# vadimkantorov/convasr

Hardware: AMD Instinct MI355X
Metric: audio-seconds/sec/node (fwd+bwd+CTC) at bs64x15s (higher is better)
Workload: dtype bf16

## Files before the change

### convasr_amd/_lib.py

```python
import ctypes
import os

import torch

_HERE = os.path.dirname(os.path.abspath(__file__))
LIB_PATH = os.environ.get('CONVASR_HIP_LIB') or os.path.join(_HERE, 'libconvasr_hip.so')

F32, BF16, I16, F16 = 0, 1, 2, 3
LOSS_SCALER_FLOATS = 8
ACT_NONE, ACT_RELU, ACT_HARDTANH, ACT_LEAKY_RELU = 0, 1, 2, 3
PACK_FWD, PACK_DGRAD = 0, 1
W_REFERENCE, W_KMAJOR = 0, 1
METRIC_CHARS, METRIC_WORDS = 0, 1
METRIC_MAX_LEN = 16383

c_int, c_i64, c_u64, c_f32, c_p = ctypes.c_int, ctypes.c_int64, ctypes.c_uint64, ctypes.c_float, ctypes.c_void_p

_SIGNATURES = dict(
	convasr_abi_version = (c_int, []),
	convasr_last_error = (ctypes.c_char_p, []),
	convasr_convert_layout = (c_int, [c_p, c_int, c_i64, c_i64, c_i64, c_p, c_int, c_i64, c_i64, c_i64, c_int, c_int, c_int, c_p]),
	convasr_signal_absmax = (c_int, [c_p, c_int, c_int, c_int, c_p, c_p]),
	convasr_logmel_fwd = (c_int, [c_p, c_int, c_p, c_p, c_p, c_int, c_p, c_p, c_p, c_int, c_int, c_int, c_int, c_int, c_f32, c_p]),
	convasr_instnorm_fwd = (c_int, [c_p, c_int, c_i64, c_i64, c_i64, c_p, c_int, c_i64, c_i64, c_i64, c_p, c_int, c_int, c_int, c_int, c_f32, c_p]),
	convasr_instnorm_running_fwd = (c_int, [c_p, c_int, c_i64, c_i64, c_i64, c_p, c_int, c_i64, c_i64, c_i64, c_int, c_int, c_int, c_int, c_f32, c_p, c_p, c_p, c_f32, c_int, c_p, c_p]),
	convasr_output_lengths = (c_int, [c_p, c_int, c_int, c_p, c_p]),
	convasr_conv_cout_pad = (c_int, [c_int]),
	convasr_pack_conv_weight = (c_int, [c_p, c_p, c_p, c_int, c_int, c_int, c_int, c_int, c_p]),
	convasr_fold2_geometry = (c_int, [c_int, c_int, ctypes.POINTER(c_int), ctypes.POINTER(c_int)]),
	convasr_fold2_pack_weight = (c_int, [c_p, c_int, c_p, c_int, c_int, c_int, c_int, c_int, c_p]),
	convasr_fold2_unfold_wgrad = (c_int, [c_p, c_p, c_int, c_int, c_int, c_int, c_int, c_int, c_p]),
	convasr_conv1d_fwd = (c_int, [c_p, c_p, c_p, c_int, c_int, c_int, c_int, c_int, c_int, c_int, c_int, c_int, c_int, c_int, c_p, c_p, c_p, c_p, c_int, c_f32, c_f32, c_p, c_p, c_p]),
	convasr_conv_stats_max_rows = (c_int, [c_int, c_int]),
	convasr_grouped_conv1d_fwd = (c_int, [c_p, c_p, c_i64, c_i64, c_i64, c_p, c_p, c_int, c_int, c_int, c_int, c_int, c_int, c_int, c_int, c_int, c_int, c_int, c_p]),
	convasr_grouped_conv1d_dgrad = (c_int, [c_p, c_p, c_p, c_i64, c_i64, c_i64, c_p, c_int, c_int, c_int, c_int, c_int, c_int, c_int, c_int, c_int, c_int, c_p]),
	convasr_grouped_conv1d_wgrad_workspace_bytes = (c_i64, [c_int, c_int, c_int, c_int, c_int]),
	convasr_grouped_conv1d_wgrad = (c_int, [c_p, c_p, c_p, c_p, c_i64, c_i64, c_i64, c_p, c_p, c_int, c_int, c_int, c_int, c_int, c_int, c_int, c_int, c_int, c_int, c_int, c_p]),
	convasr_reduce_rows = (c_int, [c_p, c_int, c_int, c_p, c_p]),
	convasr_debug_set_conv_v2 = (c_int, [c_int]),
	convasr_conv1d_wgrad_workspace_bytes = (c_i64, [c_int, c_int, c_int, c_int, c_int, c_int, c_int, c_int]),
	convasr_conv1d_wgrad = (c_int, [c_p, c_p, c_p, c_p, c_p, c_int, c_int, c_int, c_int, c_int, c_int, c_int, c_int, c_int, c_int, c_int, c_int, c_p]),
	convasr_bn_finalize = (c_int, [c_p, c_int, c_i64, c_p, c_p, c_p, c_p, c_f32, c_f32, c_p, c_p, c_p, c_p, c_int, c_p, c_p]),
	convasr_bn_eval_scale_shift = (c_int, [c_p, c_p, c_p, c_p, c_f32, c_p, c_p, c_int, c_p]),
	convasr_bn_act_fwd = (c_int, [c_p, c_p, c_int, c_p, c_p, c_int, c_p, c_p, c_p, c_int, c_f32, c_f32, c_f32, c_u64, c_u64, c_p, c_p, c_int, c_int, c_int, c_p, c_p]),
	convasr_bn_bwd_workspace_bytes = (c_i64, [c_int, c_int, c_int]),
	convasr_bn_act_bwd_reduce = (c_int, [c_p, c_p, c_p, c_int, c_p, c_p, c_p, c_p, c_int, c_p, c_p, c_p, c_p, c_p, c_p, c_int, c_f32, c_f32, c_f32, c_u64, c_u64, c_p, c_p, c_p, c_p, c_p, c_p, c_p, c_p, c_int, c_int, c_int, c_int, c_p, c_p]),
	convasr_bn_act_bwd_apply = (c_int, [c_p, c_p, c_p, c_int, c_p, c_int, c_p, c_p, c_int, c_f32, c_f32, c_f32, c_u64, c_u64, c_p, c_p, c_int, c_int, c_int, c_p, c_p]),
	convasr_bn_bwd_apply = (c_int, [c_p, c_p, c_p, c_int, c_p, c_p, c_p, c_p, c_p, c_p, c_int, c_int, c_int, c_int, c_p]),
	convasr_log_softmax_fwd = (c_int, [c_p, c_p, c_i64, c_int, c_p]),
	convasr_log_softmax_bwd = (c_int, [c_p, c_p, c_p, c_i64, c_int, c_p]),
	convasr_ctc_workspace_bytes = (c_i64, [c_int, c_int, c_int]),
	convasr_ctc_loss = (c_int, [c_p, c_p, c_p, c_p, c_p, c_p, c_p, c_int, c_int, c_int, c_int, c_int, c_p]),
	convasr_scale_rows = (c_int, [c_p, c_p, c_p, c_i64, c_p, c_int, c_i64, c_p]),
	convasr_loss_head = (c_int, [c_p, c_p, c_i64, c_p, c_int, c_f32, c_p, c_p, c_p, c_p, c_f32, c_p]),
	convasr_entropy = (c_int, [c_p, c_p, c_p, c_int, c_int, c_int, c_f32, c_p]),
	convasr_weighted_mean_entropy = (c_int, [c_p, c_p, c_p, c_int, c_int, c_int, c_int, c_f32, c_p]),
	convasr_argmax = (c_int, [c_p, c_p, c_i64, c_int, c_p]),
	convasr_sumsq_workspace_bytes = (c_i64, []),
	convasr_sumsq = (c_int, [c_p, c_i64, c_p, c_p, c_p, c_f32, c_p, c_p]),
	convasr_sgd_step = (c_int, [c_p, c_p, c_p, c_p, c_i64, c_p, c_f32, c_f32, c_f32, c_f32, c_int, c_int, c_p, c_f32, c_p, c_int, c_p, c_p, c_p, c_p]),
	convasr_adamw_step = (c_int, [c_p, c_p, c_p, c_p, c_i64, c_p, c_f32, c_f32, c_f32, c_f32, c_f32, c_f32, c_p, c_p, c_p, c_f32, c_p, c_int, c_p, c_p, c_p, c_p]),
	convasr_conv1d_dgrad_bn_reduce = (c_int, [c_p, c_p, c_p, c_int, c_int, c_int, c_int, c_int, c_int, c_int, c_int, c_int, c_p, c_p, c_p, c_p, c_p, c_int, c_f32, c_f32, c_f32, c_u64, c_u64, c_p, c_p, c_p, c_p, c_p, c_p]),
	convasr_bn_bwd_finalize = (c_int, [c_p, c_int, c_p, c_p, c_p, c_p, c_p, c_p, c_int, c_i64, c_int, c_p]),
	convasr_novograd_step = (c_int, [c_p, c_p, c_p, c_p, c_p, c_p, c_p, c_int, c_i64, c_p, c_int, c_p, c_p, c_f32, c_f32, c_f32, c_f32, c_f32, c_f32, c_int, c_int, c_p, c_p, c_f32, c_p, c_int, c_p, c_p, c_p, c_p]),
	convasr_step_begin = (c_int, [c_p, c_p]),
	convasr_conv1x1_grouped = (c_int, [c_int, c_p, c_p, c_p, c_p, c_p, c_p, c_p, c_p, c_int, c_int, c_int, ctypes.POINTER(c_int), c_p]),
	convasr_add16 = (c_int, [c_p, c_p, c_p, c_i64, c_int, c_p]),
	convasr_bn_bwd_reduce_many_workspace_bytes = (c_i64, [c_int, c_int, c_int, c_int]),
	convasr_bn_bwd_reduce_many = (c_int, [c_p, c_p, c_f32, c_p, c_int, c_p, c_p, c_p, c_p, c_p, c_p, c_p, c_p, c_p, c_int, c_int, c_int, c_int, c_p]),
	convasr_pack_dgrad_item_bytes = (c_int, []),
	convasr_pack_dgrad_grouped = (c_int, [c_p, c_int, c_int, c_p]),
	convasr_bn_finalize_grouped = (c_int, [c_int, c_p, c_int, c_i64, c_p, c_p, c_p, c_p, c_p, c_p, c_p, c_p, c_int, c_p]),
	convasr_bn_bwd_finalize_grouped = (c_int, [c_int, c_p, c_p, c_p, c_p, c_p, c_p, c_p, c_p, c_p, c_i64, c_int, c_p]),
	convasr_bn_bwd_apply_grouped = (c_int, [c_p, c_int, c_p, c_p, c_p, c_int, c_int, c_int, c_int, c_p]),
	convasr_wgrad1x1_grouped_workspace_bytes = (c_i64, [c_int, c_p, c_p, c_int, c_int]),
	convasr_wgrad1x1_grouped = (c_int, [c_int, c_p, c_p, c_p, c_p, c_p, c_p, c_p, c_p, c_int, c_int, c_int, c_p]),
	convasr_copy = (c_int, [c_p, c_p, c_i64, c_p]),
	convasr_colsum_workspace_bytes = (c_i64, [c_i64, c_int]),
	convasr_colsum = (c_int, [c_p, c_int, c_i64, c_int, c_p, c_p, c_int, c_p]),
	convasr_cast_scale = (c_int, [c_p, c_int, c_p, c_int, c_i64, c_f32, c_p]),
	convasr_bn_act_fwd_split3 = (c_int, [c_p, c_p, c_int, c_p, c_p, c_int, c_p, c_p, c_p, c_int, c_f32, c_f32, c_f32, c_u64, c_u64, c_p, c_p, c_int, c_int, c_int, c_p, c_p]),
	convasr_bn_act_bwd_apply_split3 = (c_int, [c_p, c_p, c_p, c_int, c_p, c_int, c_p, c_p, c_int, c_f32, c_f32, c_f32, c_u64, c_u64, c_p, c_p, c_int, c_int, c_int, c_p, c_p]),
	convasr_split3 = (c_int, [c_p, c_p, c_int, c_i64, c_int, c_int, c_p]),
	convasr_pack_conv_weight_split3 = (c_int, [c_p, c_int, c_p, c_p, c_int, c_int, c_int, c_int, c_int, c_p]),
	convasr_bn_act_bwd_apply_to_half = (c_int, [c_p, c_p, c_p, c_int, c_p, c_int, c_p, c_p, c_int, c_f32, c_f32, c_f32, c_u64, c_u64, c_p, c_p, c_int, c_int, c_int, c_p, c_p]),
	convasr_conv1d_fwd_splitk_plan = (c_int, [c_int, c_int, c_int, c_int, c_int, c_int, c_p]),
# ... 239 lines not shown
```

### convasr_amd/csrc/ctc.hip

```cpp
#include "common.h"

#define CTC_NEG (-1e30f)
#define CTC_DEAD (-1e29f)
#define CTC_LOG2E 1.4426950408889634f
#define CTC_LN2 0.6931471805599453
#define CTC_RENORM 8
#define CTC_RENORM_LOG2 3
#define CTC_EMPTY 0xFFFFFFFFu
#ifndef CTC_SPIN_LIMIT
#define CTC_SPIN_LIMIT (1 << 22)
#endif

__device__ __forceinline__ float lse3(float a, float b, float c) {
	const float m = fmaxf(a, fmaxf(b, c));
	const float md = __builtin_amdgcn_fmed3f(a, b, c), lo = fminf(a, fminf(b, c));
	return m + __builtin_amdgcn_logf(1.f + __builtin_amdgcn_exp2f(md - m) + __builtin_amdgcn_exp2f(lo - m));
}
__device__ __forceinline__ float lse2(float a, float b) {
	const float m = __builtin_amdgcn_fmed3f(a, b, INFINITY);
	return m + __builtin_amdgcn_logf(1.f + __builtin_amdgcn_exp2f(__builtin_amdgcn_fmed3f(a, b, -INFINITY) - m));
}

__device__ __forceinline__ float wave_shr1(float v, float fill) {
	return __builtin_bit_cast(float, __builtin_amdgcn_update_dpp(__builtin_bit_cast(int, fill), __builtin_bit_cast(int, v), 0x138, 0xf, 0xf, false));
// ... 194 lines not shown
			const int t = i / (C + 1), c = i - t * (C + 1);
			lpl[i] = c < C ? ctc_floor(lpg[(int64_t)t * C + c] * CTC_LOG2E) : CTC_NEG;
		}
	}
	__syncthreads();
	const int wave = __builtin_amdgcn_readfirstlane(threadIdx.x >> 6);
	const bool fwd = wave < 2;
	CtcSweep q;
	q.lpb = LP_LDS ? lpl : lpg;
	q.tg = targets + (int64_t)b * S_max;
	q.lat = (fwd ? alpha : beta) + (int64_t)b * T * CAP;
	q.off = offs + (((int64_t)(fwd ? 0 : 1) * B + b) * 2 + (wave & 1)) * NB;
	q.edge = edge + (fwd ? 0 : T);
	q.ecum = edge + 3 * T + (fwd ? 0 : NB);
	q.fin = fin; q.fcum = fcum + (wave & 1); q.gave_up = fcum + 2;
	q.T = T; q.C = C; q.Tb = Tb; q.L = L; q.blank = blank; q.cap = CAP; q.lane = threadIdx.x & 63;
	q.s_base = wave == 1 ? 128 * NPH : (wave == 3 ? 128 * NPL : 0);
	if (wave == 0) ctc_sweep<NPH, true, false, LP_LDS>(q);
	else if (wave == 1) ctc_sweep<NPL, true, true, LP_LDS>(q);
	else if (wave == 2) ctc_sweep<NPL, false, true, LP_LDS>(q);
	else ctc_sweep<NPH, false, false, LP_LDS>(q);
	__syncthreads();
	if (threadIdx.x == 0) {
		const float c1 = fcum[L - 1 >= 128 * NPH];
		const float l1 = fin[L - 1], l2 = L >= 2 ? fin[L - 2] + (fcum[L - 2 >= 128 * NPH] - c1) : CTC_NEG;
		const float m = fmaxf(l1, l2);
		const float rem = m + log2f(exp2f(l1 - m) + exp2f(l2 - m));
		nll[b] = fcum[2] != 0.f ? NAN : (m > CTC_DEAD ? (float)(-CTC_LN2 * ((double)c1 + (double)rem)) : INFINITY);
		tot[2 * b] = c1;
		tot[2 * b + 1] = rem;
	}
}

__global__ __launch_bounds__(256) void ctc_grad_kernel(const float* __restrict__ lp, const int64_t* __restrict__ targets, const int64_t* __restrict__ olen,
                                                       const int64_t* __restrict__ ylen, const float* __restrict__ nll, const float* __restrict__ alpha,
                                                       const float* __restrict__ beta, const float* __restrict__ offs, const float* __restrict__ tot, float* __restrict__ grad,
                                                       int B, int T, int C, int S_max, int blank, int t_per_block, int cap, int split_a, int split_b) {
	extern __shared__ float bins[];
	const int NB = T / CTC_RENORM + 1;
	const int b = blockIdx.y, lane = threadIdx.x & 63, wave = threadIdx.x >> 6;
	const int Tb = (int)olen[b], S = (int)ylen[b], L = 2 * S + 1;
	const bool feasible = nll[b] < INFINITY;
	const int64_t* tg = targets + (int64_t)b * S_max;
	float* mybins = bins + wave * C;
	const int t_begin = blockIdx.x * t_per_block, t_end = min(T, t_begin + t_per_block);
	for (int t = t_begin + wave; t < t_end; t += 4) {
		const float* row = lp + ((int64_t)b * T + t) * C;
		float* grow = grad + ((int64_t)b * T + t) * C;
		if (t >= Tb || !feasible) {
			for (int c = lane; c < C; c += 64) grow[c] = 0.f;
			continue;
		}
		for (int c = lane; c < C; c += 64) mybins[c] = 0.f;
		__builtin_amdgcn_s_waitcnt(0xc07f);
		__builtin_amdgcn_wave_barrier();
		const float* ar = alpha + ((int64_t)b * T + t) * cap;
		const float* br = beta + ((int64_t)b * T + t) * cap;
		const float* oa = offs + (int64_t)b * 2 * NB + (t >> CTC_RENORM_LOG2);
		const float* ob = offs + ((int64_t)B + b) * 2 * NB + ((Tb - 1 - t) >> CTC_RENORM_LOG2);
		const float ti = tot[2 * b], tr = tot[2 * b + 1];
		const float oa0 = oa[0] - ti, oa1 = oa[NB] - ti, ob0 = ob[0], ob1 = ob[NB];
		const float lpb = row[blank] * CTC_LOG2E;
		float blank_sum = 0.f;
		for (int s = lane; s < L; s += 64) {
			const float shift = ((s >= split_a ? oa1 : oa0) + (s >= split_b ? ob1 : ob0)) - tr;
			const float ab = ar[s] + br[s];
			if (s & 1) {
				const int c = (int)tg[s >> 1];
				atomicAdd(mybins + c, __builtin_amdgcn_exp2f(ab + (shift - row[c] * CTC_LOG2E)));
			} else blank_sum += __builtin_amdgcn_exp2f(ab + (shift - lpb));
		}
		blank_sum = wave_sum(blank_sum);
		if (lane == 0) atomicAdd(mybins + blank, blank_sum);
		__builtin_amdgcn_s_waitcnt(0xc07f);
		__builtin_amdgcn_wave_barrier();
		for (int c = lane; c < C; c += 64) grow[c] = __expf(row[c]) - mybins[c];
		__builtin_amdgcn_wave_barrier();
	}
}

static int ctc_split(int S_max, int* nph, int* npl) {
	const int pairs = (2 * S_max + 1 + 127) / 128;
	if (pairs > 16) return -1;
	const int p = pairs < 2 ? 2 : pairs;
	*nph = (p + 1) / 2;
	*npl = p / 2;
	return 0;
}

extern "C" int64_t convasr_ctc_workspace_bytes(int B, int T, int S_max) {
	int nph, npl;
	if (ctc_split(S_max, &nph, &npl) < 0) return -1;
	const int NB = T / CTC_RENORM + 1;
	return (2 * (int64_t)B * T * 128 * (nph + npl) + 4 * (int64_t)B * NB + 2 * (int64_t)B) * (int64_t)sizeof(float);
}

extern "C" int convasr_ctc_loss(const float* log_probs, const int64_t* targets, const int64_t* olen, const int64_t* ylen, float* nll, float* grad,
                                void* workspace, int B, int T, int C, int S_max, int blank, void* stream) {
	CONVASR_CHECK_ARG(log_probs && targets && olen && ylen && nll && workspace && B > 0 && T > 0 && C > 1 && S_max >= 0 && blank >= 0 && blank < C, "ctc_loss: bad arguments");
	int nph, npl;
	if (ctc_split(S_max, &nph, &npl) < 0) return convasr_fail(CONVASR_EUNSUPPORTED, "ctc_loss: target length %d > 1023", S_max);
	CONVASR_CHECK_ARG(C <= 8192, "ctc_loss: C %d > 8192", C);
	hipStream_t s = (hipStream_t)stream;
	const int NB = T / CTC_RENORM + 1, cap = 128 * (nph + npl);
	float* alpha = (float*)workspace;
	float* beta = alpha + (int64_t)B * T * cap;
	float* offs = beta + (int64_t)B * T * cap;
	float* tot = offs + 4 * (int64_t)B * NB;
	const int t_per_block = 32;
	dim3 ggrid((T + t_per_block - 1) / t_per_block, B);
	const size_t gsmem = 4 * (size_t)C * sizeof(float);
	const size_t lds_fixed = (size_t)(cap + 4 + ((3 * T + 2 * NB + 3) & ~3)) * sizeof(float), lds_lp = (size_t)T * (C + 1) * sizeof(float);
	CONVASR_CHECK_ARG(lds_fixed <= 159 * 1024, "ctc_loss: T %d too long for the edge slots", T);
	const bool in_lds = lds_fixed + lds_lp <= 159 * 1024;
#define CTC_LAUNCH(NPH, NPL, LDS) do { \
		auto kern = ctc_alpha_beta_kernel<NPH, NPL, LDS>; \
		static unsigned long long set = 0; \
		convasr_allow_160k_lds(reinterpret_cast<const void*>(kern), set); \
		hipLaunchKernelGGL(kern, dim3(B), dim3(256), lds_fixed + (LDS ? lds_lp : 0), s, log_probs, targets, olen, ylen, nll, alpha, beta, offs, tot, B, T, C, S_max, blank); \
	} while (0)
#define CTC_CASE(NPH, NPL) case NPH + NPL: if (in_lds) CTC_LAUNCH(NPH, NPL, true); else CTC_LAUNCH(NPH, NPL, false); break;
	switch (nph + npl) {
		CTC_CASE(1, 1) CTC_CASE(2, 1) CTC_CASE(2, 2) CTC_CASE(3, 2) CTC_CASE(3, 3) CTC_CASE(4, 3) CTC_CASE(4, 4)
		CTC_CASE(5, 4) CTC_CASE(5, 5) CTC_CASE(6, 5) CTC_CASE(6, 6) CTC_CASE(7, 6) CTC_CASE(7, 7) CTC_CASE(8, 7) CTC_CASE(8, 8)
	}
#undef CTC_CASE
#undef CTC_LAUNCH
	if (grad) hipLaunchKernelGGL(ctc_grad_kernel, ggrid, dim3(256), gsmem, s, log_probs, targets, olen, ylen, nll, alpha, beta, offs, tot, grad, B, T, C, S_max, blank, t_per_block, cap, 128 * nph, 128 * npl);
	CONVASR_CHECK_LAUNCH("ctc_loss");
	return 0;
}
```

### convasr_amd/functional.py

```python
import os

import torch

from . import ops, _lib

_pack_cache = {}
_param_epoch = [0]


def bump_param_epoch():
	_param_epoch[0] += 1


def param_version(w):
	return (w._version, w.data_ptr(), _param_epoch[0])


def packed_weight(w, dtype, mode):
	ver = param_version(w)
	ent = _pack_cache.get((id(w), dtype))
	if ent is not None:
		if mode == _lib.PACK_DGRAD:
			if ent['dgr_ver'] == ver:
				return ent['dgr']
# ... 1128 lines not shown
	def forward(ctx, logits):
		lp = ops.log_softmax(ops.as_cl(logits, torch.float32))
		ctx.save_for_backward(lp)
		return lp

	@staticmethod
	def backward(ctx, g):
		lp, = ctx.saved_tensors
		return ops.log_softmax_bwd(g, lp)


class CtcLossFunction(torch.autograd.Function):

	@staticmethod
	def forward(ctx, log_probs, targets, olen, ylen, blank, norm = None):
		lp = ops.as_cl(log_probs, torch.float32)
		need = log_probs.requires_grad
		nll, grad = ops.ctc_loss(lp, targets, olen, ylen, blank, need_grad = need)
		ctx.norm = norm
		if need:
			ctx.save_for_backward(grad)
		if norm is None:
			return nll
		if norm.dtype == torch.int64 and norm.ndim == 1 and norm.device == nll.device:
			return ops.scale_rows(nll, None, norm)
		return nll / norm

	@staticmethod
	def backward(ctx, g):
		grad, = ctx.saved_tensors
		return ops.scale_rows(grad, g, ctx.norm), None, None, None, None, None


def ctc_loss(log_probs, targets, olen, ylen, blank, norm = None):
	return CtcLossFunction.apply(log_probs, targets, olen, ylen, blank, norm)
```

### convasr_amd/models.py

```python
import math
import os
import typing
import weakref

import numpy as np
import torch
import torch.nn as nn

from . import ops, _lib
from . import functional as Fn
from .functional import ConvSpec

FP16_TINY = float(torch.finfo(torch.float16).tiny)



def compute_output_lengths(x, lengths_fraction = None):
	B, T = x.shape[0], x.shape[-1]
	if lengths_fraction is None:
		return torch.full((B, ), T, dtype = torch.int64, device = x.device)
	return torch.ceil(lengths_fraction * T).to(torch.int64)


def temporal_mask(x, lengths):
# ... 362 lines not shown
			assert (not self.check_time_dim_padded) or (x.shape[-1] % (32 / 2) == 0), 'Shape of input signal is not divisible by 16 '
			x = x.squeeze(1)
			x = self.frontend(x, xlen = xlen) if isinstance(self.frontend, LogFilterBankFrontend) else self.frontend(x, mask = temporal_mask(x, compute_output_lengths(x, xlen)) if xlen is not None else None)
		assert (not self.check_time_dim_padded) or (x.shape[-1] % 32 == 0), 'Shape of features after frontend is not divisible by 32'
		assert x.ndim == 3
		if self.normalize_features is not None:
			conv0 = self.backbone[0].conv[0][-1]
			pad_even = (self.compute_dtype in ops.HALF_DTYPES or (self.split_dtype is not None and self.training and torch.is_grad_enabled())) and x.shape[-1] % 2 == 1 and Fn.Fold2.wants_even_input(conv0.weight.shape, _spec_of(conv0), x.shape[-1])
			x = self.normalize_features(x, xlen = xlen, out_dtype = self.compute_dtype, pad_time_to = 2 if pad_even else 1)
		else:
			x = ops.as_cl(x, self.compute_dtype)

		residual = []
		n = len(self.backbone)
		for i, block in enumerate(self.backbone):
			x = block(x, residual = residual, lengths_fraction = xlen)
			if i >= n - self.num_epilogue_modules - 1:
				residual = []
			elif self.residual == 'dense':
				residual = residual + [x]
			elif self.residual:
				residual = [x]
			else:
				residual = []

		logits = self.decoder(x)
		if y is not None and ylen is not None and self.training and torch.is_grad_enabled():
			cached = getattr(self, '_dgrad_weights', None)
			if cached is None or cached[0] != Fn.structure_epoch():
				convs = [c[-1] for blk in self.modules() if isinstance(blk, ConvBn1d) for c in blk.conv] + [c for blk in self.modules() if isinstance(blk, ConvBn1d) for c in blk.conv_residual if isinstance(c, nn.Conv1d)]
				cached = self._dgrad_weights = (Fn.structure_epoch(), [c.weight for c in convs[1:] if c.stride[0] == 1])
			if self.split_dtype is None:
				Fn.prepack_dgrad_weights(cached[1], self.compute_dtype)
		log_probs = [Fn.LogSoftmaxFunction.apply(l) for l in logits]
		olen = [ops.output_lengths(xlen, l.shape[0], l.shape[-1], l.device) for l in logits]
		aux = {}
		if y is not None and ylen is not None:
			loss = [Fn.ctc_loss(lp, y[:, i], olen[i], ylen[:, i], lp.shape[1] - 1, norm = ylen[:, 0]) for i, lp in enumerate(log_probs)]
			heads = loss if not self.bpe_only else loss[1:]
			if not heads:
				aux = dict(loss = torch.zeros_like(loss[0]))
			else:
				aux = dict(loss = heads[0] if len(heads) == 1 else sum(heads[1:], heads[0]))
		return self.dict(logits = logits, log_probs = log_probs, olen = olen, **aux)

	def freeze(self, backbone = 0, decoder0 = False, frontend = False):
		targets = list(self.backbone[:backbone]) if backbone else []
		if decoder0:
			targets.append(self.decoder[0])
		if frontend and self.frontend is not None:
			targets.append(self.frontend)
		for part in targets:
			for bn in part.modules():
				if isinstance(bn, nn.modules.batchnorm._BatchNorm):
					bn.eval()
					bn.train = lambda training: None
			for p in part.parameters():
				p.requires_grad = False

	def fuse_conv_bn_eval(self, K = None):
		self._dgrad_weights = None
		for block in self.backbone[:K]:
			block.fuse_conv_bn_eval()

	def set_temporal_mask_mode(self, enabled):
		for module in self.modules():
			module.temporal_mask = enabled
# ... 145 lines not shown
```

### convasr_amd/ops.py

```python
import math
import os

import ctypes

import torch

from . import _lib
from ._lib import call, ptr, stream_ptr, dtype_code, require_cuda

HALF_DTYPES = (torch.bfloat16, torch.float16)

ACT_CODES = dict(none = _lib.ACT_NONE, relu = _lib.ACT_RELU, hardtanh = _lib.ACT_HARDTANH, leaky_relu = _lib.ACT_LEAKY_RELU)


def act_args(nonlinearity):
	if nonlinearity is None:
		return _lib.ACT_NONE, 0.0, 0.0
	name = nonlinearity[0]
	if name == 'relu':
		return _lib.ACT_RELU, 0.0, 0.0
	if name == 'hardtanh':
		return _lib.ACT_HARDTANH, float(nonlinearity[1]), float(nonlinearity[2])
	if name == 'leaky_relu':
		return _lib.ACT_LEAKY_RELU, float(nonlinearity[1]) if len(nonlinearity) > 1 else 0.01, 0.0
# ... 530 lines not shown
		assert y.dtype == torch.float32 and planes in HALF_DTYPES and out is None
		dy3 = empty_cl(B, 3 * C, T, planes, y.device)
		_lib.timed('hbm:bn_act_bwd_apply_kernel', 0.0, lambda: call('convasr_bn_act_bwd_apply_split3', ptr(dz_or_g), ptr(y), ptr(dy3), dtype_code(planes), ptr(coef), int(from_dz), ptr(scale), ptr(shift), act[0], act[1], act[2], float(dropout_p), int(seed), int(offset), step_key, ptr(xlen), B, T, C, ptr(gate), stream_ptr()), nbytes = float(B * T * C * 14))
		return dy3
	dy = out if out is not None else empty_cl(B, C, T, y.dtype, y.device)
	_lib.timed('hbm:bn_act_bwd_apply_kernel', 0.0, lambda: call('convasr_bn_act_bwd_apply', ptr(dz_or_g), ptr(y), ptr(dy), dtype_code(y.dtype), ptr(coef), int(from_dz), ptr(scale), ptr(shift), act[0], act[1], act[2], float(dropout_p), int(seed), int(offset), step_key, ptr(xlen), B, T, C, ptr(gate), stream_ptr()), nbytes = float(B * T * C * y.element_size() * 3))
	return dy


def bn_bwd_apply(g, y, gamma, mean, invstd, sums, dgamma = None, dbeta = None, accumulate = False, need_dy = True, inplace = True):
	B, C, T = y.shape
	dy = (g if inplace else empty_cl(B, C, T, y.dtype, y.device)) if need_dy else None
	call('convasr_bn_bwd_apply', ptr(g), ptr(y), ptr(dy), dtype_code(y.dtype), ptr(gamma), ptr(mean), ptr(invstd), ptr(sums), ptr(dgamma), ptr(dbeta), int(accumulate), B, T, C, stream_ptr())
	return dy



def log_softmax(logits):
	B, C, T = logits.shape
	assert is_cl(logits) and logits.dtype == torch.float32
	out = empty_cl(B, C, T, torch.float32, logits.device)
	call('convasr_log_softmax_fwd', ptr(logits), ptr(out), B * T, C, stream_ptr())
	return out


def log_softmax_bwd(grad_lp, log_probs):
	B, C, T = log_probs.shape
	grad_lp = as_cl(grad_lp, torch.float32)
	out = empty_cl(B, C, T, torch.float32, log_probs.device)
	call('convasr_log_softmax_bwd', ptr(grad_lp), ptr(log_probs), ptr(out), B * T, C, stream_ptr())
	return out


def ctc_loss(log_probs, targets, olen, ylen, blank, need_grad = True):
	B, C, T = log_probs.shape
	assert is_cl(log_probs) and log_probs.dtype == torch.float32
	dev = log_probs.device
	targets = targets.to(device = dev, dtype = torch.int64).contiguous()
	if targets.ndim == 1:
		targets = targets.view(B, -1)
	olen = olen.to(device = dev, dtype = torch.int64).contiguous()
	ylen = ylen.to(device = dev, dtype = torch.int64).contiguous()
	S_max = targets.shape[1]
	nbytes = _lib.load().convasr_ctc_workspace_bytes(B, T, S_max)
	if nbytes < 0:
		raise _lib.ConvasrHipError(f'ctc_loss: target length {S_max} unsupported')
	ws = workspace(nbytes, dev, 'ctc')
	nll = torch.empty(B, dtype = torch.float32, device = dev)
	grad = empty_cl(B, C, T, torch.float32, dev) if need_grad else None
	call('convasr_ctc_loss', ptr(log_probs), ptr(targets), ptr(olen), ptr(ylen), ptr(nll), ptr(grad), ptr(ws), B, T, C, S_max, blank, stream_ptr())
	return nll, grad


def scale_rows(grad, gscale, gdiv = None):
	B = grad.shape[0]
	out = torch.empty_like(grad)
	assert gdiv is None or (gdiv.dtype == torch.int64 and gdiv.ndim == 1 and gdiv.shape[0] == B and gdiv.device == grad.device)
	call('convasr_scale_rows', ptr(grad), None if gscale is None else ptr(gscale.to(torch.float32).contiguous()), ptr(gdiv), 0 if gdiv is None else gdiv.stride(0), ptr(out), B, grad.numel() // B, stream_ptr())
	return out


def loss_head(loss_vec, ylen_col, ent = None, accumulate_iterations = 1, need_grad = True, loss_scaler = None, metric_scale = 1.0):
	require_cuda(loss_vec)
	B = loss_vec.shape[0]
	lv = loss_vec.detach().to(torch.float32).contiguous()
	assert ylen_col.dtype == torch.int64 and ylen_col.ndim == 1 and ylen_col.shape[0] == B and ylen_col.device == lv.device
	out3 = torch.empty(3, dtype = torch.float32, device = lv.device)
	gvec = torch.empty(B, dtype = torch.float32, device = lv.device) if need_grad else None
	skipped = torch.empty(1, dtype = torch.bool, device = lv.device)
	ent = None if ent is None else ent.detach().to(torch.float32).contiguous()
	call('convasr_loss_head', ptr(lv), ptr(ylen_col), ylen_col.stride(0), ptr(ent), B, float(accumulate_iterations), ptr(out3), ptr(gvec), ptr(skipped), ptr(loss_scaler), float(metric_scale), stream_ptr())
	return out3, gvec, skipped


def entropy(log_probs, olen = None, eps = 1e-9):
	B, C, T = log_probs.shape
	lp = as_cl(log_probs, torch.float32)
	ent = torch.empty(B, dtype = torch.float32, device = lp.device)
	ol = None if olen is None else olen.to(device = lp.device, dtype = torch.int64).contiguous()
	call('convasr_entropy', ptr(lp), ptr(ol), ptr(ent), B, T, C, float(eps), stream_ptr())
	return ent


def weighted_mean_entropy(log_probs, olen = None, eps = 1e-9, eps_id = -1):
# ... 477 lines not shown
```

### include/convasr_hip.h

```cpp
#ifndef CONVASR_HIP_H
#define CONVASR_HIP_H

#include <stdint.h>

#ifdef __cplusplus
extern "C" {
#endif

#define CONVASR_ABI_VERSION 10

enum { CONVASR_F32 = 0, CONVASR_BF16 = 1, CONVASR_I16 = 2, CONVASR_F16 = 3 };
enum { CONVASR_ACT_NONE = 0, CONVASR_ACT_RELU = 1, CONVASR_ACT_HARDTANH = 2, CONVASR_ACT_LEAKY_RELU = 3 };
enum { CONVASR_OK = 0, CONVASR_EINVAL = -1, CONVASR_ELAUNCH = -2, CONVASR_EUNSUPPORTED = -3 };

int convasr_abi_version(void);
const char* convasr_last_error(void);


int convasr_convert_layout(const void* src, int src_dtype, int64_t src_sb, int64_t src_sc, int64_t src_st,
                           void* dst, int dst_dtype, int64_t dst_sb, int64_t dst_sc, int64_t dst_st,
                           int B, int C, int T, void* stream);


int convasr_signal_absmax(const void* signal, int signal_dtype, int B, int T, float* absmax, void* stream);
// ... 67 lines not shown
int convasr_bn_eval_scale_shift(const float* gamma, const float* beta, const float* running_mean, const float* running_var,
                                float eps, float* scale, float* shift, int C, void* stream);

int convasr_bn_act_fwd(const void* y, void* z, int dtype, const float* scale, const float* shift,
                       int n_res, const void* const* res, const float* const* rscale, const float* const* rshift,
                       int act, float act_lo, float act_hi, float dropout_p, uint64_t seed, uint64_t offset, const uint64_t* step_key,
                       const float* xlen, int B, int T, int C, uint8_t* gate, void* stream);

int64_t convasr_bn_bwd_workspace_bytes(int B, int T, int C);
int convasr_bn_act_bwd_reduce(const void* dz, const void* y, void* g, int dtype, const float* scale, const float* shift,
                              const float* mean, const float* invstd,
                              int n_res, const void* const* res, const float* const* rscale, const float* const* rshift,
                              const float* const* rmean, const float* const* rinvstd, double* const* rsums,
                              int act, float act_lo, float act_hi, float dropout_p, uint64_t seed, uint64_t offset, const uint64_t* step_key,
                              const float* xlen, double* sums, void* workspace, const float* gamma, float* coef, float* dgamma, float* dbeta,
                              int accumulate, int B, int T, int C, const uint8_t* gate, void* stream);

int convasr_bn_act_bwd_apply(const void* dz_or_g, const void* y, void* dy, int dtype, const float* coef, int from_dz,
                             const float* scale, const float* shift, int act, float act_lo, float act_hi, float dropout_p,
                             uint64_t seed, uint64_t offset, const uint64_t* step_key, const float* xlen, int B, int T, int C, const uint8_t* gate, void* stream);

int convasr_bn_bwd_apply(const void* g, const void* y, void* dy, int dtype, const float* gamma, const float* mean,
                         const float* invstd, const double* sums, float* dgamma, float* dbeta, int accumulate,
                         int B, int T, int C, void* stream);


int convasr_log_softmax_fwd(const float* logits, float* log_probs, int64_t rows, int C, void* stream);
int convasr_log_softmax_bwd(const float* grad_lp, const float* log_probs, float* dlogits, int64_t rows, int C, void* stream);

int64_t convasr_ctc_workspace_bytes(int B, int T, int S_max);
int convasr_ctc_loss(const float* log_probs, const int64_t* targets, const int64_t* olen, const int64_t* ylen,
                     float* nll, float* grad, void* workspace, int B, int T, int C, int S_max, int blank, void* stream);
int convasr_scale_rows(const float* grad, const float* gscale, const int64_t* gdiv, int64_t gdiv_stride, float* out, int B, int64_t per_b, void* stream);

int convasr_loss_head(const float* loss_vec, const int64_t* ylen, int64_t ylen_stride, const float* entropy, int B, float accumulate_iterations, float* out3,
                      float* grad_loss_vec, unsigned char* skipped, const float* loss_scaler, float metric_scale, void* stream);

#define CONVASR_LOSS_SCALER_FLOATS 8

int convasr_entropy(const float* log_probs, const int64_t* olen, float* ent, int B, int T, int C, float eps, void* stream);
int convasr_weighted_mean_entropy(const float* log_probs, const int64_t* olen, float* out, int B, int T, int C, int eps_id, float eps, void* stream);
int convasr_argmax(const float* log_probs, int64_t* idx, int64_t rows, int C, void* stream);


int64_t convasr_sumsq_workspace_bytes(void);
int convasr_sumsq(const float* g, int64_t n, double* sumsq, void* workspace, float* norm_out, float norm_scale, const float* loss_scaler, void* stream);
int convasr_sgd_step(float* p, const float* g, float* buf, float* grad_out, int64_t n, const double* sumsq, float max_norm,
                     float lr, float momentum, float weight_decay, int nesterov, int first, const float* loss_gate, float grad_scale,
                     void* p16, int p16_dtype, const float* scaler_in, float* scaler_out, const float* lr_dev, void* stream);
int convasr_adamw_step(float* p, const float* g, float* exp_avg, float* exp_avg_sq, int64_t n, const double* sumsq, float max_norm, float lr,
                       float beta1, float beta2, float eps, float weight_decay, const float* step_in, float* step_out, const float* loss_gate,
                       float grad_scale, void* p16, int p16_dtype, const float* scaler_in, float* scaler_out, const float* lr_dev, void* stream);

int convasr_conv1d_dgrad_bn_reduce(const void* dy, const void* packed_dgrad, void* dx, int dtype, int B, int Cout, int Cin, int T_dy, int T_dx, int K,
                                   int dil, int pad, const void* bn_y, const float* bn_scale, const float* bn_shift, const float* bn_mean,
                                   const float* bn_invstd, int bn_act, float bn_act_lo, float bn_act_hi, float dropout_p, uint64_t seed,
                                   uint64_t offset, const uint64_t* step_key, const float* bn_xlen, double* bn_sums, int* bn_rows, const uint8_t* bn_gate, void* stream);
int convasr_bn_bwd_finalize(const double* sums, int sums_rows, const float* gamma, const float* mean, const float* invstd, float* coef,
                            float* dgamma, float* dbeta, int accumulate, int64_t n, int C, void* stream);


int convasr_conv1x1_grouped(int n, const void* const* x, const void* const* w, void* const* y, const float* const* bias, double* const* stats,
                            const int* cin, const int* cout, const int* accumulate, int dtype, int B, int T, int* stats_rows, void* stream);
int64_t convasr_wgrad1x1_grouped_workspace_bytes(int n, const int* cin, const int* cout, int B, int T);
int convasr_wgrad1x1_grouped(int n, const void* const* x, const void* const* dy, float* const* dw, float* const* zero, const int* cin, const int* cout,
                             const int* accumulate, void* workspace, int dtype, int B, int T, void* stream);
// ... 156 lines not shown
```

Before: 58780.

## Fuse CTC gradient, row scaling and log-softmax backward into one kernel

```diff
diff --git a/convasr_amd/_lib.py b/convasr_amd/_lib.py
--- a/convasr_amd/_lib.py
+++ b/convasr_amd/_lib.py
@@ -52,6 +52,7 @@
 	convasr_ctc_workspace_bytes = (c_i64, [c_int, c_int, c_int]),
 	convasr_ctc_loss = (c_int, [c_p, c_p, c_p, c_p, c_p, c_p, c_p, c_int, c_int, c_int, c_int, c_int, c_p]),
 	convasr_scale_rows = (c_int, [c_p, c_p, c_p, c_i64, c_p, c_int, c_i64, c_p]),
+	convasr_ctc_grad_logits = (c_int, [c_p, c_p, c_p, c_p, c_p, c_p, c_p, c_p, c_i64, c_p, c_int, c_int, c_int, c_int, c_int, c_p]),
 	convasr_loss_head = (c_int, [c_p, c_p, c_i64, c_p, c_int, c_f32, c_p, c_p, c_p, c_p, c_f32, c_p]),
 	convasr_entropy = (c_int, [c_p, c_p, c_p, c_int, c_int, c_int, c_f32, c_p]),
 	convasr_weighted_mean_entropy = (c_int, [c_p, c_p, c_p, c_int, c_int, c_int, c_int, c_f32, c_p]),
diff --git a/convasr_amd/csrc/ctc.hip b/convasr_amd/csrc/ctc.hip
--- a/convasr_amd/csrc/ctc.hip
+++ b/convasr_amd/csrc/ctc.hip
@@ -296,6 +296,121 @@
 		__builtin_amdgcn_wave_barrier();
 	}
 }
+
+#define CTCG_LP(c) (row[c] * CTC_LOG2E)
+__global__ __launch_bounds__(256) void ctc_grad_logits_kernel(const float* __restrict__ lp, const int64_t* __restrict__ targets, const int64_t* __restrict__ olen,
+                                                              const int64_t* __restrict__ ylen, const float* __restrict__ nll, const float* __restrict__ alpha,
+                                                              const float* __restrict__ beta, const float* __restrict__ offs, const float* __restrict__ tot,
+                                                              const float* __restrict__ gscale, const int64_t* __restrict__ gdiv, int64_t gdiv_stride, float* __restrict__ dlogits,
+                                                              int B, int T, int C, int S_max, int blank, int frames, int cap, int split_a, int split_b) {
+	extern __shared__ __attribute__((aligned(16))) float cg_smem[];
+	const int SC = cap >> 1, CP = (C + 4) & ~3, CR = (C + 3) & ~3;
+	int* const pk = reinterpret_cast<int*>(cg_smem);
+	int* const cst = pk + SC;
+	float* const rowl = cg_smem + SC + CP;
+	float* const prob = rowl + 4 * CR;
+	int* const cls = reinterpret_cast<int*>(prob);
+	float* const stage = prob + 4 * SC;
+	const int NB = T / CTC_RENORM + 1;
+	const int b = blockIdx.y, tid = threadIdx.x, lane = tid & 63, wave = tid >> 6;
+	const int Tb = (int)olen[b], S = max(0, min((int)ylen[b], S_max)), L = 2 * S + 1;
+	const bool feasible = nll[b] < INFINITY;
+	const int64_t* tg = targets + (int64_t)b * S_max;
+	const int t_begin = blockIdx.x * frames, nf = min(T, t_begin + frames) - t_begin;
+	if (feasible && t_begin < Tb) {
+		for (int i = tid; i < SC; i += 256) cls[i] = i < S ? min(max((int)tg[i], 0), C - 1) : 0;
+		for (int c = tid; c < CP; c += 256) cst[c] = 0;
+		__syncthreads();
+		for (int i = tid; i < S; i += 256) atomicAdd(cst + cls[i], 1);
+		__syncthreads();
+		if (wave == 0) {
+			int v[4], sum = 0;
+#pragma unroll
+			for (int k = 0; k < 4; ++k) { v[k] = 4 * lane + k < C ? cst[4 * lane + k] : 0; sum += v[k]; }
+			int incl = sum;
+#pragma unroll
+			for (int o = 1; o < 64; o <<= 1) { const int up = __shfl_up(incl, o, 64); if (lane >= o) incl += up; }
+			int run = incl - sum;
+#pragma unroll
+			for (int k = 0; k < 4; ++k) { if (4 * lane + k < C) cst[4 * lane + k] = run; run += v[k]; }
+			if (lane == 63) cst[C] = incl;
+		}
+		__syncthreads();
+		for (int i = tid; i < SC; i += 256) {
+			int word = 0;
+			if (i < S) {
+				const int c = cls[i];
+				int rank = 0;
+				for (int j = 0; j < i; ++j) rank += cls[j] == c;
+				word = (cst[c] + rank) << 8 | c;
+			}
+			pk[i] = word;
+		}
+		__syncthreads();
+	}
+	const float s0 = gscale ? gscale[b] : 1.f;
+	const float scale = gdiv ? s0 / (float)gdiv[b * gdiv_stride] : s0;
+	float* const myrow = rowl + wave * CR;
+	float* const myprob = prob + wave * SC;
+	for (int f = wave; f < nf; f += 4) {
+		const int t = t_begin + f;
+		const float* row = lp + ((int64_t)b * T + t) * C;
+		float* srow = stage + f * C;
+		const bool live = t < Tb && feasible;
+		float blank_sum = 0.f;
+		if (live) {
+			for (int c = lane; c < C; c += 64) myrow[c] = CTCG_LP(c);
+			__builtin_amdgcn_s_waitcnt(0xc07f);
+			__builtin_amdgcn_wave_barrier();
+			const float* ar = alpha + ((int64_t)b * T + t) * cap;
+			const float* br = beta + ((int64_t)b * T + t) * cap;
+			const float* oa = offs + (int64_t)b * 2 * NB + (t >> CTC_RENORM_LOG2);
+			const float* ob = offs + ((int64_t)B + b) * 2 * NB + ((Tb - 1 - t) >> CTC_RENORM_LOG2);
+			const float ti = tot[2 * b], tr = tot[2 * b + 1];
+			const float oa0 = oa[0] - ti, oa1 = oa[NB] - ti, ob0 = ob[0], ob1 = ob[NB];
+			const float lpb = myrow[blank];
+			for (int s = 4 * lane; s < L; s += 256) {
+				const float4 a4 = *reinterpret_cast<const float4*>(ar + s), b4 = *reinterpret_cast<const float4*>(br + s);
+				const int2 w = *reinterpret_cast<const int2*>(pk + (s >> 1));
+				const float shift = ((s >= split_a ? oa1 : oa0) + (s >= split_b ? ob1 : ob0)) - tr;
+				blank_sum += __builtin_amdgcn_exp2f((a4.x + b4.x) + (shift - lpb));
+				if (s + 1 < L) myprob[w.x >> 8] = __builtin_amdgcn_exp2f((a4.y + b4.y) + (shift - myrow[w.x & 255]));
+				if (s + 2 < L) blank_sum += __builtin_amdgcn_exp2f((a4.z + b4.z) + (shift - lpb));
+				if (s + 3 < L) myprob[w.y >> 8] = __builtin_amdgcn_exp2f((a4.w + b4.w) + (shift - myrow[w.y & 255]));
+			}
+			blank_sum = wave_sum(blank_sum);
+			__builtin_amdgcn_s_waitcnt(0xc07f);
+			__builtin_amdgcn_wave_barrier();
+		}
+		float gsum = 0.f;
+		for (int c = lane; c < C; c += 64) {
+			float g = 0.f;
+			if (live) {
+				float p = 0.f;
+				for (int k = cst[c], e = cst[c + 1]; k < e; ++k) p += myprob[k];
+				if (c == blank) p += blank_sum;
+				g = __expf(row[c]) - p;
+			}
+			g *= scale;
+			srow[c] = g;
+			gsum += g;
+		}
+		gsum = wave_sum(gsum);
+		for (int c = lane; c < C; c += 64) srow[c] = srow[c] - expf(row[c]) * gsum;
+		__builtin_amdgcn_wave_barrier();
+	}
+	__syncthreads();
+	const int64_t e0 = ((int64_t)b * T + t_begin) * C;
+	float* dst = dlogits + e0;
+	const int n = nf * C, head = min(n, (int)((4 - (e0 & 3)) & 3)), n4 = (n - head) >> 2, done = head + 4 * n4;
+	if (tid < head) dst[tid] = stage[tid];
+	for (int i = tid; i < n4; i += 256) {
+		const float* sp = stage + head + 4 * i;
+		*reinterpret_cast<float4*>(dst + head + 4 * i) = make_float4(sp[0], sp[1], sp[2], sp[3]);
+	}
+	if (tid < n - done) dst[done + tid] = stage[done + tid];
+}
+#undef CTCG_LP
 
 static int ctc_split(int S_max, int* nph, int* npl) {
 	const int pairs = (2 * S_max + 1 + 127) / 128;
@@ -348,3 +463,22 @@
 	CONVASR_CHECK_LAUNCH("ctc_loss");
 	return 0;
 }
+
+extern "C" int convasr_ctc_grad_logits(const float* log_probs, const int64_t* targets, const int64_t* olen, const int64_t* ylen, const float* nll, const void* workspace,
+                                       const float* gscale, const int64_t* gdiv, int64_t gdiv_stride, float* dlogits, int B, int T, int C, int S_max, int blank, void* stream) {
+	CONVASR_CHECK_ARG(log_probs && targets && olen && ylen && nll && workspace && dlogits && B > 0 && B <= 65535 && T > 0 && C > 1 && S_max >= 0 && blank >= 0 && blank < C, "ctc_grad_logits: bad arguments");
+	CONVASR_CHECK_ARG((((uintptr_t)workspace | (uintptr_t)dlogits) & 15) == 0, "ctc_grad_logits: workspace and dlogits must be 16-byte aligned");
+	int nph, npl;
+	if (ctc_split(S_max, &nph, &npl) < 0) return convasr_fail(CONVASR_EUNSUPPORTED, "ctc_grad_logits: target length %d > 1023", S_max);
+	if (C > 256) return convasr_fail(CONVASR_EUNSUPPORTED, "ctc_grad_logits: C %d > 256 (convasr_ctc_loss, convasr_scale_rows and convasr_log_softmax_bwd take any C)", C);
+	const int NB = T / CTC_RENORM + 1, cap = 128 * (nph + npl), frames = C <= 128 ? 32 : 16;
+	const float* alpha = (const float*)workspace;
+	const float* beta = alpha + (int64_t)B * T * cap;
+	const float* offs = beta + (int64_t)B * T * cap;
+	const float* tot = offs + 4 * (int64_t)B * NB;
+	const size_t smem = ((size_t)(cap / 2) * 5 + ((C + 4) & ~3) + 4 * ((C + 3) & ~3) + (size_t)frames * C) * sizeof(float);
+	hipLaunchKernelGGL(ctc_grad_logits_kernel, dim3((T + frames - 1) / frames, B), dim3(256), smem, (hipStream_t)stream, log_probs, targets, olen, ylen, nll, alpha, beta, offs, tot,
+	                   gscale, gdiv, gdiv_stride, dlogits, B, T, C, S_max, blank, frames, cap, 128 * nph, 128 * npl);
+	CONVASR_CHECK_LAUNCH("ctc_grad_logits");
+	return 0;
+}
diff --git a/convasr_amd/functional.py b/convasr_amd/functional.py
--- a/convasr_amd/functional.py
+++ b/convasr_amd/functional.py
@@ -1184,5 +1184,31 @@
 		return ops.scale_rows(grad, g, ctx.norm), None, None, None, None, None
 
 
+class LogSoftmaxCtcLossFunction(torch.autograd.Function):
+
+	@staticmethod
+	def forward(ctx, logits, lp, targets, olen, ylen, blank, norm = None):
+		nll, ctx.state = ops.ctc_loss(lp, targets, olen, ylen, blank, need_grad = False, return_state = True)
+		ctx.norm = norm
+		return nll if norm is None else ops.scale_rows(nll, None, norm)
+
+	@staticmethod
+	def backward(ctx, g):
+		return ops.ctc_grad_logits(ctx.state, g, ctx.norm), None, None, None, None, None, None
+
+
+FUSED_CTC_GRAD = [os.environ.get('CONVASR_NO_FUSED_CTC_GRAD', '0') != '1']
+
+
+def log_softmax(logits):
+	lp = LogSoftmaxFunction.apply(logits)
+	lp.__dict__['_convasr_logits'] = (logits, lp._version)
+	return lp
+
+
 def ctc_loss(log_probs, targets, olen, ylen, blank, norm = None):
+	src = log_probs.__dict__.get('_convasr_logits')
+	if (FUSED_CTC_GRAD[0] and src is not None and src[1] == log_probs._version and torch.is_grad_enabled() and src[0].requires_grad and log_probs.shape[1] <= ops.CTC_GRAD_LOGITS_MAX_C
+			and (norm is None or (norm.dtype == torch.int64 and norm.ndim == 1 and norm.device == log_probs.device))):
+		return LogSoftmaxCtcLossFunction.apply(src[0], log_probs.detach(), targets, olen, ylen, blank, norm)
 	return CtcLossFunction.apply(log_probs, targets, olen, ylen, blank, norm)
diff --git a/convasr_amd/models.py b/convasr_amd/models.py
--- a/convasr_amd/models.py
+++ b/convasr_amd/models.py
@@ -418,7 +418,7 @@
 				cached = self._dgrad_weights = (Fn.structure_epoch(), [c.weight for c in convs[1:] if c.stride[0] == 1])
 			if self.split_dtype is None:
 				Fn.prepack_dgrad_weights(cached[1], self.compute_dtype)
-		log_probs = [Fn.LogSoftmaxFunction.apply(l) for l in logits]
+		log_probs = [Fn.log_softmax(l) for l in logits]
 		olen = [ops.output_lengths(xlen, l.shape[0], l.shape[-1], l.device) for l in logits]
 		aux = {}
 		if y is not None and ylen is not None:
diff --git a/convasr_amd/ops.py b/convasr_amd/ops.py
--- a/convasr_amd/ops.py
+++ b/convasr_amd/ops.py
@@ -586,7 +586,7 @@
 	return out
 
 
-def ctc_loss(log_probs, targets, olen, ylen, blank, need_grad = True):
+def ctc_loss(log_probs, targets, olen, ylen, blank, need_grad = True, return_state = False):
 	B, C, T = log_probs.shape
 	assert is_cl(log_probs) and log_probs.dtype == torch.float32
 	dev = log_probs.device
@@ -603,7 +603,27 @@
 	nll = torch.empty(B, dtype = torch.float32, device = dev)
 	grad = empty_cl(B, C, T, torch.float32, dev) if need_grad else None
 	call('convasr_ctc_loss', ptr(log_probs), ptr(targets), ptr(olen), ptr(ylen), ptr(nll), ptr(grad), ptr(ws), B, T, C, S_max, blank, stream_ptr())
+	_ctc_fills[0] += 1
+	ws.__dict__['_convasr_ctc_fill'] = _ctc_fills[0]
+	if return_state:
+		return nll, (log_probs, targets, olen, ylen, nll, ws, _ctc_fills[0], blank)
 	return nll, grad
+
+
+CTC_GRAD_LOGITS_MAX_C = 256
+_ctc_fills = [0]
+
+
+def ctc_grad_logits(state, gscale, gdiv = None):
+	log_probs, targets, olen, ylen, nll, ws, fill, blank = state
+	if ws.__dict__.get('_convasr_ctc_fill') != fill:
+		nll, (_, _, _, _, _, ws, _, _) = ctc_loss(log_probs, targets, olen, ylen, blank, need_grad = False, return_state = True)
+	B, C, T = log_probs.shape
+	assert gdiv is None or (gdiv.dtype == torch.int64 and gdiv.ndim == 1 and gdiv.shape[0] == B and gdiv.device == log_probs.device)
+	out = empty_cl(B, C, T, torch.float32, log_probs.device)
+	call('convasr_ctc_grad_logits', ptr(log_probs), ptr(targets), ptr(olen), ptr(ylen), ptr(nll), ptr(ws), None if gscale is None else ptr(gscale.to(torch.float32).contiguous()),
+		ptr(gdiv), 0 if gdiv is None else gdiv.stride(0), ptr(out), B, T, C, targets.shape[1], blank, stream_ptr())
+	return out
 
 
 def scale_rows(grad, gscale, gdiv = None):
diff --git a/include/convasr_hip.h b/include/convasr_hip.h
--- a/include/convasr_hip.h
+++ b/include/convasr_hip.h
@@ -123,6 +123,9 @@
 int convasr_ctc_loss(const float* log_probs, const int64_t* targets, const int64_t* olen, const int64_t* ylen,
                      float* nll, float* grad, void* workspace, int B, int T, int C, int S_max, int blank, void* stream);
 int convasr_scale_rows(const float* grad, const float* gscale, const int64_t* gdiv, int64_t gdiv_stride, float* out, int B, int64_t per_b, void* stream);
+int convasr_ctc_grad_logits(const float* log_probs, const int64_t* targets, const int64_t* olen, const int64_t* ylen, const float* nll,
+                            const void* workspace, const float* gscale, const int64_t* gdiv, int64_t gdiv_stride, float* dlogits,
+                            int B, int T, int C, int S_max, int blank, void* stream);
 
 int convasr_loss_head(const float* loss_vec, const int64_t* ylen, int64_t ylen_stride, const float* entropy, int B, float accumulate_iterations, float* out3,
                       float* grad_loss_vec, unsigned char* skipped, const float* loss_scaler, float metric_scale, void* stream);
```

Result: no change. 58860, median of 4 (+0.1%).

## Replace CTC grad LDS atomics with per-class gather via sorted target order

Applied to the files above, without the earlier changes.

```diff
diff --git a/convasr_amd/csrc/ctc.hip b/convasr_amd/csrc/ctc.hip
--- a/convasr_amd/csrc/ctc.hip
+++ b/convasr_amd/csrc/ctc.hip
@@ -250,50 +250,134 @@
 	}
 }
 
+template <int J, bool SMALL>
 __global__ __launch_bounds__(256) void ctc_grad_kernel(const float* __restrict__ lp, const int64_t* __restrict__ targets, const int64_t* __restrict__ olen,
                                                        const int64_t* __restrict__ ylen, const float* __restrict__ nll, const float* __restrict__ alpha,
                                                        const float* __restrict__ beta, const float* __restrict__ offs, const float* __restrict__ tot, float* __restrict__ grad,
                                                        int B, int T, int C, int S_max, int blank, int t_per_block, int cap, int split_a, int split_b) {
-	extern __shared__ float bins[];
-	const int NB = T / CTC_RENORM + 1;
+	extern __shared__ __attribute__((aligned(16))) float bins[];
+	constexpr int NREG = 8;
+	const int NB = T / CTC_RENORM + 1, H = cap >> 1;
 	const int b = blockIdx.y, lane = threadIdx.x & 63, wave = threadIdx.x >> 6;
-	const int Tb = (int)olen[b], S = (int)ylen[b], L = 2 * S + 1;
-	const bool feasible = nll[b] < INFINITY;
+	const int Tb = (int)olen[b], S = min((int)ylen[b], min(S_max, H - 1)), L = 2 * S + 1;
 	const int64_t* tg = targets + (int64_t)b * S_max;
-	float* mybins = bins + wave * C;
 	const int t_begin = blockIdx.x * t_per_block, t_end = min(T, t_begin + t_per_block);
+	if (!(nll[b] < INFINITY) || t_begin >= Tb) {
+		for (int t = t_begin + wave; t < t_end; t += 4)
+			for (int c = lane; c < C; c += 64) grad[((int64_t)b * T + t) * C + c] = 0.f;
+		return;
+	}
+	int* const tgl = reinterpret_cast<int*>(bins);
+	int* const order = tgl + H;
+	int* const stcnt = order + H;
+	float* const terms = reinterpret_cast<float*>(stcnt + 128) + wave * H;
+	float* const mybins = bins + wave * C;
+	int st = 0, cnt = 0, oreg[NREG];
+	if (SMALL) {
+		for (int i = threadIdx.x; i < H; i += blockDim.x) tgl[i] = i < S ? (int)tg[i] : -1;
+		__syncthreads();
+		if (wave == 0) {
+			int n = 0;
+			for (int i = 0; i < S; i += 4) {
+				const int4 v = *reinterpret_cast<const int4*>(tgl + i);
+				n += (v.x == lane) + (v.y == lane) + (v.z == lane) + (v.w == lane);
+			}
+			int incl = n;
+			for (int o = 1; o < 64; o <<= 1) {
+				const int v = __shfl_up(incl, o, 64);
+				if (lane >= o) incl += v;
+			}
+			stcnt[lane] = incl - n;
+			stcnt[64 + lane] = n;
+		}
+		__syncthreads();
+		for (int i = threadIdx.x; i < S; i += blockDim.x) {
+			const int c = tgl[i];
+			int r = 0;
+			for (int j = 0; j < i; j += 4) {
+				const int4 v = *reinterpret_cast<const int4*>(tgl + j);
+				r += (v.x == c) + (j + 1 < i && v.y == c) + (j + 2 < i && v.z == c) + (j + 3 < i && v.w == c);
+			}
+			if ((unsigned)c < 64u) order[stcnt[c] + r] = i;
+		}
+		__syncthreads();
+		st = stcnt[lane];
+		cnt = stcnt[64 + lane];
+#pragma unroll
+		for (int k = 0; k < NREG; ++k) oreg[k] = k < cnt ? order[st + k] : 0;
+	}
+	int c0[J], c1[J];
+#pragma unroll
+	for (int j = 0; j < J; ++j) {
+		const int s = 4 * lane + 256 * j;
+		c0[j] = s + 1 < L ? (int)tg[s >> 1] : 0;
+		c1[j] = s + 3 < L ? (int)tg[(s >> 1) + 1] : 0;
+	}
+	const float ti = tot[2 * b], tr = tot[2 * b + 1];
 	for (int t = t_begin + wave; t < t_end; t += 4) {
 		const float* row = lp + ((int64_t)b * T + t) * C;
 		float* grow = grad + ((int64_t)b * T + t) * C;
-		if (t >= Tb || !feasible) {
+		if (t >= Tb) {
 			for (int c = lane; c < C; c += 64) grow[c] = 0.f;
 			continue;
 		}
-		for (int c = lane; c < C; c += 64) mybins[c] = 0.f;
-		__builtin_amdgcn_s_waitcnt(0xc07f);
-		__builtin_amdgcn_wave_barrier();
-		const float* ar = alpha + ((int64_t)b * T + t) * cap;
-		const float* br = beta + ((int64_t)b * T + t) * cap;
+		const float* ar = alpha + ((int64_t)b * T + t) * cap + 4 * lane;
+		const float* br = beta + ((int64_t)b * T + t) * cap + 4 * lane;
+		ctc_f4 ab[J];
+#pragma unroll
+		for (int j = 0; j < J; ++j) ab[j] = 4 * lane + 256 * j < L ? *reinterpret_cast<const ctc_f4*>(ar + 256 * j) : ctc_f4{0.f, 0.f, 0.f, 0.f};
+#pragma unroll
+		for (int j = 0; j < J; ++j) if (4 * lane + 256 * j < L) ab[j] += *reinterpret_cast<const ctc_f4*>(br + 256 * j);
+		const float rl = SMALL && lane < C ? row[lane] : 0.f;
 		const float* oa = offs + (int64_t)b * 2 * NB + (t >> CTC_RENORM_LOG2);
 		const float* ob = offs + ((int64_t)B + b) * 2 * NB + ((Tb - 1 - t) >> CTC_RENORM_LOG2);
-		const float ti = tot[2 * b], tr = tot[2 * b + 1];
 		const float oa0 = oa[0] - ti, oa1 = oa[NB] - ti, ob0 = ob[0], ob1 = ob[NB];
-		const float lpb = row[blank] * CTC_LOG2E;
+		if (!SMALL) {
+			for (int c = lane; c < C; c += 64) mybins[c] = 0.f;
+			__builtin_amdgcn_s_waitcnt(0xc07f);
+			__builtin_amdgcn_wave_barrier();
+		}
+		const float lpb = (SMALL ? __shfl(rl, blank, 64) : row[blank]) * CTC_LOG2E;
 		float blank_sum = 0.f;
-		for (int s = lane; s < L; s += 64) {
+#pragma unroll
+		for (int j = 0; j < J; ++j) {
+			const int s = 4 * lane + 256 * j;
 			const float shift = ((s >= split_a ? oa1 : oa0) + (s >= split_b ? ob1 : ob0)) - tr;
-			const float ab = ar[s] + br[s];
-			if (s & 1) {
-				const int c = (int)tg[s >> 1];
-				atomicAdd(mybins + c, __builtin_amdgcn_exp2f(ab + (shift - row[c] * CTC_LOG2E)));
-			} else blank_sum += __builtin_amdgcn_exp2f(ab + (shift - lpb));
+			const float r0 = (SMALL ? __shfl(rl, c0[j], 64) : (s + 1 < L ? row[c0[j]] : 0.f)) * CTC_LOG2E;
+			const float r1 = (SMALL ? __shfl(rl, c1[j], 64) : (s + 3 < L ? row[c1[j]] : 0.f)) * CTC_LOG2E;
+			const float e1 = __builtin_amdgcn_exp2f(ab[j][1] + (shift - r0)), e3 = __builtin_amdgcn_exp2f(ab[j][3] + (shift - r1));
+			if (s < L) blank_sum += __builtin_amdgcn_exp2f(ab[j][0] + (shift - lpb));
+			if (s + 2 < L) blank_sum += __builtin_amdgcn_exp2f(ab[j][2] + (shift - lpb));
+			if (SMALL) {
+				if (s + 1 < L) *reinterpret_cast<ctc_f2*>(terms + (s >> 1)) = ctc_f2{e1, e3};
+			} else {
+				if (s + 1 < L) atomicAdd(mybins + c0[j], e1);
+				if (s + 3 < L) atomicAdd(mybins + c1[j], e3);
+			}
 		}
 		blank_sum = wave_sum(blank_sum);
-		if (lane == 0) atomicAdd(mybins + blank, blank_sum);
-		__builtin_amdgcn_s_waitcnt(0xc07f);
-		__builtin_amdgcn_wave_barrier();
-		for (int c = lane; c < C; c += 64) grow[c] = __expf(row[c]) - mybins[c];
-		__builtin_amdgcn_wave_barrier();
+		if (SMALL) {
+			__builtin_amdgcn_fence(__ATOMIC_RELEASE, "wavefront");
+			__builtin_amdgcn_wave_barrier();
+			__builtin_amdgcn_fence(__ATOMIC_ACQUIRE, "wavefront");
+			float post = lane == blank ? blank_sum : 0.f;
+#pragma unroll
+			for (int k = 0; k < NREG; ++k) {
+				const float v = terms[oreg[k]];
+				post += k < cnt ? v : 0.f;
+			}
+			for (int k = NREG; k < cnt; ++k) post += terms[order[st + k]];
+			if (lane < C) grow[lane] = __expf(rl) - post;
+			__builtin_amdgcn_fence(__ATOMIC_RELEASE, "wavefront");
+			__builtin_amdgcn_wave_barrier();
+			__builtin_amdgcn_fence(__ATOMIC_ACQUIRE, "wavefront");
+		} else {
+			if (lane == 0) atomicAdd(mybins + blank, blank_sum);
+			__builtin_amdgcn_s_waitcnt(0xc07f);
+			__builtin_amdgcn_wave_barrier();
+			for (int c = lane; c < C; c += 64) grow[c] = __expf(row[c]) - mybins[c];
+			__builtin_amdgcn_wave_barrier();
+		}
 	}
 }
 
@@ -327,7 +411,8 @@
 	float* tot = offs + 4 * (int64_t)B * NB;
 	const int t_per_block = 32;
 	dim3 ggrid((T + t_per_block - 1) / t_per_block, B);
-	const size_t gsmem = 4 * (size_t)C * sizeof(float);
+	const bool small = C <= 64;
+	const size_t gsmem = (small ? 6 * (size_t)(cap / 2) + 128 : 4 * (size_t)C) * sizeof(float);
 	const size_t lds_fixed = (size_t)(cap + 4 + ((3 * T + 2 * NB + 3) & ~3)) * sizeof(float), lds_lp = (size_t)T * (C + 1) * sizeof(float);
 	CONVASR_CHECK_ARG(lds_fixed <= 159 * 1024, "ctc_loss: T %d too long for the edge slots", T);
 	const bool in_lds = lds_fixed + lds_lp <= 159 * 1024;
@@ -344,7 +429,13 @@
 	}
 #undef CTC_CASE
 #undef CTC_LAUNCH
-	if (grad) hipLaunchKernelGGL(ctc_grad_kernel, ggrid, dim3(256), gsmem, s, log_probs, targets, olen, ylen, nll, alpha, beta, offs, tot, grad, B, T, C, S_max, blank, t_per_block, cap, 128 * nph, 128 * npl);
+	if (grad) {
+#define CTC_GRAD_(J, SMALL) hipLaunchKernelGGL((ctc_grad_kernel<J, SMALL>), ggrid, dim3(256), gsmem, s, log_probs, targets, olen, ylen, nll, alpha, beta, offs, tot, grad, B, T, C, S_max, blank, t_per_block, cap, 128 * nph, 128 * npl)
+#define CTC_GRAD(J) case J: if (small) CTC_GRAD_(J, true); else CTC_GRAD_(J, false); break;
+		switch ((cap + 255) / 256) { CTC_GRAD(1) CTC_GRAD(2) CTC_GRAD(3) CTC_GRAD(4) CTC_GRAD(5) CTC_GRAD(6) CTC_GRAD(7) CTC_GRAD(8) }
+#undef CTC_GRAD
+#undef CTC_GRAD_
+	}
 	CONVASR_CHECK_LAUNCH("ctc_loss");
 	return 0;
 }
```

Result: no change. 58900 before, 59090 after (median of 6 runs) (+0.3%).
